# SaeedRahmani/MPC_for_AV_at_Intersection

Hardware: AMD Instinct MI355X
Metric: MPC timesteps/sec (whole node), N=20 horizon, 8-agent intersection, batch=4096 (higher is better)
Workload: dtype f64

## Files before the change

### mpc_for_av_at_intersection_amd/csrc/mpcx_prepare.hip

```cpp
#include "mpcx_common.h"
#include "mpcx_predict_core.h"
#include <cmath>

namespace mpcx {

struct RefArgs {
    mpcx_mpc_params p;
    int B;
    const double *state, *path, *path_v;
    const int32_t *path_off, *path_len;
    double dl;
    int32_t *target_ind;
    double *xref;
    uint8_t *re;
    const double *ov;
    long ov_stride;
    const int32_t *bin_cnt, *keyslot;
    int32_t *order;
    const int32_t *near, *near_tidx;
    const int32_t *stop_idx;
    double v_ref;
    int32_t *len_seen;
    const int32_t *done;
    int32_t *queue_len;
};

constexpr int PREP_WAVES = 4;
constexpr int WIN_AGENTS = 8;
static_assert(WIN_AGENTS <= WAVE, "one lane per agent in parts 1 and 2");
template <bool RETIRE>
__global__ __launch_bounds__(64 * PREP_WAVES) void ref_window_kernel(RefArgs a) {
    __shared__ int s_first[MPCX_ORDER_COPIES][MPCX_ORDER_BINS];
    const int lane = threadIdx.x & 63, wave = threadIdx.x >> 6;
    const int T = a.p.T, W = T + 1;
    const int b0 = ((int)blockIdx.x * PREP_WAVES + wave) * WIN_AGENTS;
    const int nag = a.B - b0 < WIN_AGENTS ? a.B - b0 : WIN_AGENTS;
    const bool own = lane < nag;
    const int b = own ? b0 + lane : 0;
    bool gone = !own;
    if constexpr (RETIRE) gone = gone || a.done[b] != 0;
    const int off = a.path_off[b], n = a.path_len[b];
    const double x = a.state[4 * b], y = a.state[4 * b + 1], v = a.state[4 * b + 2];
    const int start = a.target_ind[b];
    const int ks = a.order ? a.keyslot[b] : 0;
    const int hs = a.near ? a.near[3 * b] : -1, hm = a.near ? a.near[3 * b + 1] : -1, hl = a.near ? a.near[3 * b + 2] : -1;
    const int hint = a.near ? a.near_tidx[b] : -1;
    const int stop_at = a.stop_idx ? a.stop_idx[b] : MPCX_NO_STOP;
    if (a.order) {
        static_assert(MPCX_ORDER_BINS == 64, "one bin per lane");
        if (wave == 0) {
            int cnt[MPCX_ORDER_COPIES], c = 0;
#pragma unroll
            for (int q = 0; q < MPCX_ORDER_COPIES; q++) { cnt[q] = a.bin_cnt[q * MPCX_ORDER_BINS + lane]; c += cnt[q]; }
            int sfx = c;
#pragma unroll
            for (int d = 1; d < 64; d <<= 1) { const int o = __shfl_down(sfx, d); sfx += lane + d < 64 ? o : 0; }
            if constexpr (RETIRE) { if (blockIdx.x == 0 && lane == 0) *a.queue_len = sfx; }
            int first = sfx - c;
#pragma unroll
            for (int q = 0; q < MPCX_ORDER_COPIES; q++) { s_first[q][lane] = first; first += cnt[q]; }
        }
        __syncthreads();
        if (!gone)
            a.order[s_first[b % MPCX_ORDER_COPIES][(ks >> 24) & (MPCX_ORDER_BINS - 1)] + (ks & 0xFFFFFF)] = b;
    }
    int s = -1;
    bool scan = false;
    if (!gone) {
        if (hm >= 0 && start >= hs && hl >= start && hm < n) s = hint;
        else scan = !(start < 0 || n <= 0);
    }
    for (unsigned long long todo = __ballot(scan); todo; todo &= todo - 1) {
        const int i = __ffsll((long long)todo) - 1;
        const int r = nearest_index_in_direction(a.path + 3 * (size_t)__shfl(off, i), __shfl(n, i), __shfl(start, i), __shfl(x, i), __shfl(y, i), lane);
        s = lane == i ? r : s;
    }
    int stop = 0x7fffffff;
    if (!gone) {
        a.target_ind[b] = s;
        stop = stop_at == MPCX_NO_STOP ? stop : stop_at;
        if (a.stop_idx && a.len_seen) a.len_seen[b] = n;
    }
    const int G = 64 / W;
    const int g = lane / W, t = lane - g * W;
    for (int base = 0; base < nag; base += G) {
        const int i = base + g;
        const bool on = g < G && i < nag;
        const int from = on ? i : 0;
        const bool skip = __shfl((int)gone, from) != 0;
        const int si = __shfl(s, from), ni = __shfl(n, from), oi = __shfl(off, from), stopi = __shfl(stop, from);
        const double vi = __shfl(v, from);
        if (!on || skip) continue;
        const int bi = b0 + i;
        const double *path = a.path + 3 * (size_t)oi;
        const double *pv = a.path_v ? a.path_v + (size_t)oi : nullptr;
        double *xr = a.xref + (size_t)bi * 4 * W;
        uint8_t *re = a.re + (size_t)bi * W;
        if (si < 0) {
            xr[t] = 0; xr[W + t] = 0; xr[2 * W + t] = 0; xr[3 * W + t] = 0; re[t] = 0;
            continue;
        }
        const double ov = vi > 10.0 / 3.6 ? vi : 10.0 / 3.6;
        const double step = __dmul_rn(fabs(ov), a.p.dt);
        const double *ovp = a.ov ? a.ov + (size_t)bi * a.ov_stride : nullptr;
        double travel = ovp ? __dmul_rn(fabs(ovp[0]), a.p.dt) : step;
        for (int k = 1; k <= t; k++) travel = __dadd_rn(travel, ovp ? __dmul_rn(fabs(ovp[k]), a.p.dt) : step);
        long long idx = (long long)rint(__ddiv_rn(travel, a.dl)) + si;
        if (idx > ni - 1) idx = ni - 1;
        xr[0 * W + t] = path[3 * idx];
        xr[1 * W + t] = path[3 * idx + 1];
        xr[2 * W + t] = idx >= stopi ? 0.0 : (pv ? pv[idx] : a.v_ref);
        xr[3 * W + t] = path[3 * idx + 2];
        re[t] = (idx == ni - 1);
    }
}

__device__ __forceinline__ double plant_tan(const mpcx_mpc_params &p, double delta) {
    return tan(fmax(fmin(delta, p.max_steer), -p.max_steer));
}
__device__ __forceinline__ double plant_rate_xy(double v, double cs) {
#pragma clang fp contract(off)
    return v * cs;
}
__device__ __forceinline__ double plant_rate_th(const mpcx_mpc_params &p, double v, double tn) {
#pragma clang fp contract(off)
    return (v / p.L) * tn;
}
__device__ __forceinline__ double plant_euler(const mpcx_mpc_params &p, double acc, double rate) { return fma(rate, p.dt, acc); }
__device__ __forceinline__ double plant_speed(const mpcx_mpc_params &p, double v, double a) {
    return fmax(fmin(plant_euler(p, v, a), p.max_speed), p.min_speed);
}
__device__ __forceinline__ void plant_step(const mpcx_mpc_params &p, double &x, double &y, double &v, double &th,
                                           double a, double delta) {
    const double tn = plant_tan(p, delta);
    double s, c;
    sincos(th, &s, &c);
    x = plant_euler(p, x, plant_rate_xy(v, c));
    y = plant_euler(p, y, plant_rate_xy(v, s));
    th = plant_euler(p, th, plant_rate_th(p, v, tn));
    v = plant_speed(p, v, a);
}

struct RollArgs {
    mpcx_mpc_params p;
    int B;
    const double *state, *u_warm;
    double *xbar;
    const int32_t *done;
};

constexpr int ROLL_GROUP = 4, ROLL_BLOCK = 256, ROLL_AGENTS = ROLL_BLOCK / ROLL_GROUP;
static_assert(WAVE % ROLL_GROUP == 0 && ROLL_BLOCK % WAVE == 0, "whole groups per wavefront");
inline size_t rollout_lds(int T) { return ROLL_AGENTS * (4 * (size_t)(T + 1) + 1) * sizeof(double); }
__device__ __forceinline__ void rollout_group(const mpcx_mpc_params &p, double x, double y, double v, double th, const double *oa, int j, double *xb) {
    constexpr int G = ROLL_GROUP;
    const int T = p.T, W = T + 1;
    if (j == 0) { xb[0] = x; xb[W] = y; xb[2 * W] = v; xb[3 * W] = th; }
    const auto euler = [&](double acc, double rate) { return plant_euler(p, acc, rate); };
    const auto speed = [&](double vv, double acc) { return plant_speed(p, vv, acc); };
    for (int t0 = 0; t0 < T; t0 += G) {
        const int t = t0 + j;
        const bool in = t < T;
        const double ai = oa && in ? oa[t] : 0.0, di = oa && in ? oa[T + t] : 0.0;
        const double tn = plant_tan(p, di);
        const double v0 = v, th0 = th;
        const double vn = group_chain<G>(v, ai, j, speed);
        const double vt = group_prev<G>(vn, v0, j);
        const double thn = group_chain<G>(th, plant_rate_th(p, vt, tn), j, euler);
        const double tht = group_prev<G>(thn, th0, j);
        double s, c;
        sincos(tht, &s, &c);
        const double xn = group_chain<G>(x, plant_rate_xy(vt, c), j, euler);
        const double yn = group_chain<G>(y, plant_rate_xy(vt, s), j, euler);
        if (in) { xb[t + 1] = xn; xb[W + t + 1] = yn; xb[2 * W + t + 1] = vn; xb[3 * W + t + 1] = thn; }
    }
}
template <bool RETIRE>
__global__ __launch_bounds__(ROLL_BLOCK) void rollout_kernel(RollArgs a) {
    constexpr int G = ROLL_GROUP;
    extern __shared__ double s_roll[];
    const int T = a.p.T, W = T + 1;
    const int RS = 4 * W + 1;
    auto s_x = [&](int row) -> double * { return s_roll + (size_t)row * RS; };
    const int b0 = (int)blockIdx.x * ROLL_AGENTS;
    const int n = a.B - b0 < ROLL_AGENTS ? a.B - b0 : ROLL_AGENTS;
    const int r = (int)threadIdx.x / G, j = (int)threadIdx.x % G;
    bool gone = r >= n;
    if constexpr (RETIRE) gone = gone || a.done[b0 + r] != 0;
    if (j == 0) s_x(r)[4 * W] = gone ? 1.0 : 0.0;
    if (!gone) {
        const int b = b0 + r;
        double x = a.state[4 * b], y = a.state[4 * b + 1], v = a.state[4 * b + 2], th = a.state[4 * b + 3];
        rollout_group(a.p, x, y, v, th, a.u_warm ? a.u_warm + (size_t)b * 2 * T : nullptr, j, s_x(r));
    }
    __syncthreads();
    double *out = a.xbar + (size_t)b0 * 4 * W;
    for (int i = threadIdx.x; i < n * 4 * W; i += ROLL_BLOCK) {
        const int row = i / (4 * W);
        if (!RETIRE || s_x(row)[4 * W] == 0.0) out[i] = s_x(row)[i - row * 4 * W];
    }
}


struct PlantArgs {
    mpcx_mpc_params p;
    int B;
    double *state;
    double *u;
    const int32_t *status;
    double *applied;
    const mpcx_qp_tuning *tune;
    const int32_t *iters;
    unsigned long long *stats;
    int has_stats;
    int32_t *zero_bins, *zero_ticket;
    const int32_t *done;
};

__device__ __forceinline__ void plant_stats(unsigned long long *stats, int b, bool in, int it, bool bad) {
    int s_it = it, s_bad = bad ? 1 : 0, s_n = in ? 1 : 0, s_mx = it;
#pragma unroll
    for (int d = 32; d >= 1; d >>= 1) {
        s_it += __shfl_xor(s_it, d, WAVE); s_bad += __shfl_xor(s_bad, d, WAVE); s_n += __shfl_xor(s_n, d, WAVE);
        const int o = __shfl_xor(s_mx, d, WAVE); s_mx = o > s_mx ? o : s_mx;
    }
    if ((threadIdx.x & 63) == 0) {
        unsigned long long *w = stats + 4 * (size_t)(b >> 6);
        w[0] += (unsigned long long)s_n; w[1] += (unsigned long long)s_it; w[2] += (unsigned long long)s_bad;
        if ((unsigned long long)s_mx > w[3]) w[3] = (unsigned long long)s_mx;
    }
}

__global__ __launch_bounds__(256) void plant_kernel(PlantArgs a) {
    if (a.zero_bins && blockIdx.x == 0) {
        for (int i = threadIdx.x; i < MPCX_ORDER_COPIES * MPCX_ORDER_BINS; i += blockDim.x) a.zero_bins[i] = 0;
        if (threadIdx.x < MPCX_TICKET_WORDS) a.zero_ticket[threadIdx.x] = 0;
    }
    const int b = blockIdx.x * blockDim.x + threadIdx.x;
    const bool gone = a.done && b < a.B && a.done[b] != 0;
    if (a.has_stats) {
        const bool in = b < a.B && !gone;
        plant_stats(a.stats, b, in, in ? a.iters[b] : 0, in && a.status[b] != MPCX_QP_OPTIMAL);
    }
    if (b >= a.B || gone) return;
    const int T = a.p.T;
    double di = a.applied[2 * b], ai;
    const bool ok = !a.status || a.status[b] == MPCX_QP_OPTIMAL;
    if (ok) { di = a.u[(size_t)b * 2 * T + T]; ai = a.u[(size_t)b * 2 * T]; }
    else {
        ai = a.tune ? a.tune[b].max_decel : a.p.max_decel;
        for (int t = 0; t < 2 * T; t++) a.u[(size_t)b * 2 * T + t] = 0.0;
    }
    a.applied[2 * b] = di; a.applied[2 * b + 1] = ai;
    double x = a.state[4 * b], y = a.state[4 * b + 1], v = a.state[4 * b + 2], th = a.state[4 * b + 3];
    plant_step(a.p, x, y, v, th, ai, di);
    a.state[4 * b] = x; a.state[4 * b + 1] = y; a.state[4 * b + 2] = v; a.state[4 * b + 3] = th;
}

struct HeadArgs {
    mpcx_mpc_params p;
    mpcx_interaction_params ip;
    int B;
    double *state, *applied, *u;
    double *xbar, *obs6, *pred;
    const int32_t *status, *iters;
    const mpcx_qp_tuning *tune;
    unsigned long long *stats;
    int32_t *zero_bins, *zero_ticket;
};

constexpr int HEAD_BLOCK = ROLL_BLOCK + WAVE;
static_assert(ROLL_AGENTS == WAVE, "the prediction wavefront holds the workgroup's agents one per lane; its statistics slot is plant_kernel's");
template <bool PLANT>
__global__ __launch_bounds__(HEAD_BLOCK) void head_kernel(HeadArgs a) {
    constexpr int G = ROLL_GROUP;
    extern __shared__ double s_roll[];
    const int T = a.p.T, W = T + 1;
    const int RS = 4 * W + 1;
    const int tid = (int)threadIdx.x;
    const bool pred_wave = tid >= ROLL_BLOCK;
    const int b0 = (int)blockIdx.x * ROLL_AGENTS;
    const int n = a.B - b0 < ROLL_AGENTS ? a.B - b0 : ROLL_AGENTS;
    const int r = pred_wave ? tid - ROLL_BLOCK : tid / G, j = tid % G;
    const bool in = r < n;
    const int b = b0 + (in ? r : 0);
    double x = a.state[4 * b], y = a.state[4 * b + 1], v = a.state[4 * b + 2], th = a.state[4 * b + 3];
    double di = 0.0, ai = 0.0;
    bool failed = false;
    if constexpr (PLANT) {
        if (a.zero_bins && blockIdx.x == 0) {
            for (int i = tid; i < MPCX_ORDER_COPIES * MPCX_ORDER_BINS; i += HEAD_BLOCK) a.zero_bins[i] = 0;
            if (tid < MPCX_TICKET_WORDS) a.zero_ticket[tid] = 0;
        }
        failed = a.status[b] != MPCX_QP_OPTIMAL;
        const int it = pred_wave && in ? a.iters[b] : 0;
        di = a.applied[2 * b];
        if (!failed) { di = a.u[(size_t)b * 2 * T + T]; ai = a.u[(size_t)b * 2 * T]; }
        else { ai = a.p.max_decel; if (a.tune) ai = a.tune[b].max_decel; }
        plant_step(a.p, x, y, v, th, ai, di);
        __syncthreads();
        if (pred_wave) {
            plant_stats(a.stats, b0 + r, in, it, in && failed);
            if (in) {
                if (failed) for (int t = 0; t < 2 * T; t++) a.u[(size_t)b * 2 * T + t] = 0.0;
                a.applied[2 * b] = di; a.applied[2 * b + 1] = ai;
                a.state[4 * b] = x; a.state[4 * b + 1] = y; a.state[4 * b + 2] = v; a.state[4 * b + 3] = th;
            }
        }
    } else if (pred_wave) {
        di = a.applied[2 * b]; ai = a.applied[2 * b + 1];
    }
    if (pred_wave) {
        if (!in) return;
        double *row = a.obs6 + 6 * (size_t)b;
        row[0] = x; row[1] = y; row[2] = v; row[3] = th; row[4] = ai; row[5] = di;
        predict_row<false>(a.ip, x, y, v, th, ai, di, nullptr, a.pred + (size_t)b * a.ip.pred_steps * 4);
        return;
    }
    if (in) rollout_group(a.p, x, y, v, th, failed ? nullptr : a.u + (size_t)b * 2 * T, j, s_roll + (size_t)r * RS);
    __builtin_amdgcn_fence(__ATOMIC_RELEASE, "wavefront");
    __builtin_amdgcn_wave_barrier();
    __builtin_amdgcn_fence(__ATOMIC_ACQUIRE, "wavefront");
    constexpr int ROWS = WAVE / G;
    const int lane = tid & 63, r0 = (tid >> 6) * ROWS;
    const int nr = n - r0 < ROWS ? n - r0 : ROWS;
    double *out = a.xbar + (size_t)(b0 + r0) * 4 * W;
    for (int i = lane; i < nr * 4 * W; i += WAVE) {
        const int row = i / (4 * W);
        out[i] = s_roll[(size_t)(r0 + row) * RS + (i - row * 4 * W)];
    }
}

}

extern "C" int32_t mpcx_mpc_prepare_batch(mpcx_ctx *ctx, int32_t B, const double *state, const double *u_warm,
                                          const double *path_xyyaw, const double *path_v, const int32_t *path_off,
                                          const int32_t *path_len, double dl, int32_t *target_ind, double *xref, uint8_t *reaches_end, double *xbar) {
    return mpcx_mpc_prepare_batch_ov(ctx, B, state, u_warm, path_xyyaw, path_v, path_off, path_len, dl, target_ind, nullptr, 0, xref, reaches_end, xbar);
}

extern "C" int32_t mpcx_mpc_prepare_batch_ov(mpcx_ctx *ctx, int32_t B, const double *state, const double *u_warm,
                                             const double *path_xyyaw, const double *path_v, const int32_t *path_off,
                                             const int32_t *path_len, double dl, int32_t *target_ind, const double *ov, int64_t ov_stride,
                                             double *xref, uint8_t *reaches_end, double *xbar) {
    return mpcx_window_enqueue(ctx, B, state, u_warm, path_xyyaw, path_v, path_off, path_len, dl, target_ind, ov, ov_stride, xref, reaches_end, xbar, {});
}

extern "C" int32_t mpcx_mpc_prepare_batch_stop(mpcx_ctx *ctx, int32_t B, const double *state, const double *u_warm,
                                               const double *path_xyyaw, const double *path_v, const int32_t *path_off,
                                               const int32_t *path_len, double dl, int32_t *target_ind, const double *ov, int64_t ov_stride,
                                               const int32_t *stop_idx, double v_ref, int32_t *len_seen,
                                               double *xref, uint8_t *reaches_end, double *xbar) {
    mpcx_window_extras wx;
    wx.stop_idx = stop_idx; wx.v_ref = v_ref; wx.len_seen = len_seen;
    return mpcx_window_enqueue(ctx, B, state, u_warm, path_xyyaw, path_v, path_off, path_len, dl, target_ind, ov, ov_stride, xref, reaches_end, xbar, wx);
}

int32_t mpcx_window_enqueue(mpcx_ctx *ctx, int32_t B, const double *state, const double *u_warm, const double *path_xyyaw, const double *path_v,
                            const int32_t *path_off, const int32_t *path_len, double dl, int32_t *target_ind, const double *ov, int64_t ov_stride,
                            double *xref, uint8_t *reaches_end, double *xbar, const mpcx_window_extras &x) {
    if (!ctx) return MPCX_E_INVALID;
    if (!ctx->have_mpc) return mpcx_fail(ctx, MPCX_E_INVALID, "mpcx_set_mpc_params has not been called");
    if (B == 0) return MPCX_OK;
    if (B < 0 || !state || !path_xyyaw || !path_off || !path_len || !target_ind || !xref || !reaches_end || !xbar || !(dl > 0))
        return mpcx_fail(ctx, MPCX_E_INVALID, "mpc_prepare_batch: null pointer, negative batch or dl <= 0");
    if (ov && ov_stride < (int64_t)ctx->mpc.T + 1)
        return mpcx_fail(ctx, MPCX_E_INVALID, "mpc_prepare_batch_ov: ov_stride %lld is smaller than T + 1", (long long)ov_stride);
    if (x.stop_idx && !std::isfinite(x.v_ref))
        return mpcx_fail(ctx, MPCX_E_INVALID, "mpc_prepare_batch_stop: v_ref is not finite");
    mpcx::RefArgs ra{ctx->mpc, B, state, path_xyyaw, path_v, path_off, path_len, dl, target_ind, xref, reaches_end, ov, (long)ov_stride,
                     x.scatter ? ctx->bins : nullptr, x.scatter ? ctx->bins + MPCX_ORDER_COPIES * MPCX_ORDER_BINS : nullptr, x.scatter ? ctx->order : nullptr,
                     x.near, x.near ? x.tidx : nullptr, x.stop_idx, x.stop_idx ? x.v_ref : 0.0, x.stop_idx ? x.len_seen : nullptr,
                     x.done, x.queue_len};
    const bool retire = x.done != nullptr;
    if (retire && (!x.scatter || !x.queue_len))
        return mpcx_fail(ctx, MPCX_E_INVALID, "mpc_prepare_batch: retirement needs the queue order built beside the window selection");
    const bool forked = x.rollout_forked;
    if (x.rollout_done) {
        constexpr int per_block = mpcx::PREP_WAVES * mpcx::WIN_AGENTS;
        const dim3 wgrid((B + per_block - 1) / per_block), wblock(64 * mpcx::PREP_WAVES);
        if (retire) hipLaunchKernelGGL(mpcx::ref_window_kernel<true>, wgrid, wblock, 0, ctx->stream, ra);
        else hipLaunchKernelGGL(mpcx::ref_window_kernel<false>, wgrid, wblock, 0, ctx->stream, ra);
        return mpcx_check_launch(ctx, "prepare kernels");
    }
    if (!forked) {
        int32_t rc = mpcx_rollout_fork(ctx, B, state, u_warm, xbar, x.done);
        if (rc != MPCX_OK) return rc;
    }
    if (forked && hipStreamWaitEvent(ctx->stream, ctx->ev_join, 0) != hipSuccess)
        return mpcx_fail(ctx, MPCX_E_LAUNCH, "mpc_prepare_batch: cannot join the side stream");
    constexpr int per_block = mpcx::PREP_WAVES * mpcx::WIN_AGENTS;
    const dim3 wgrid((B + per_block - 1) / per_block), wblock(64 * mpcx::PREP_WAVES);
    if (retire) hipLaunchKernelGGL(mpcx::ref_window_kernel<true>, wgrid, wblock, 0, ctx->stream, ra);
    else hipLaunchKernelGGL(mpcx::ref_window_kernel<false>, wgrid, wblock, 0, ctx->stream, ra);
    if (!forked && hipStreamWaitEvent(ctx->stream, ctx->ev_join, 0) != hipSuccess)
        return mpcx_fail(ctx, MPCX_E_LAUNCH, "mpc_prepare_batch: cannot join the side stream");
    return mpcx_check_launch(ctx, "prepare kernels");
}

int32_t mpcx_rollout_fork(mpcx_ctx *ctx, int32_t B, const double *state, const double *u_warm, double *xbar, const int32_t *done) {
    mpcx::RollArgs ro{ctx->mpc, B, state, u_warm, xbar, done};
    if (hipEventRecord(ctx->ev_fork, ctx->stream) != hipSuccess || hipStreamWaitEvent(ctx->side, ctx->ev_fork, 0) != hipSuccess)
        return mpcx_fail(ctx, MPCX_E_LAUNCH, "mpc_prepare_batch: cannot fork the side stream");
    const size_t roll_lds = mpcx::rollout_lds(ctx->mpc.T);
    const dim3 rgrid((B + mpcx::ROLL_AGENTS - 1) / mpcx::ROLL_AGENTS), rblock(mpcx::ROLL_BLOCK);
    if (done) hipLaunchKernelGGL(mpcx::rollout_kernel<true>, rgrid, rblock, roll_lds, ctx->side, ro);
    else hipLaunchKernelGGL(mpcx::rollout_kernel<false>, rgrid, rblock, roll_lds, ctx->side, ro);
    const int32_t rc = mpcx_check_launch(ctx, "rollout_kernel");
    if (rc != MPCX_OK) return rc;
    if (hipEventRecord(ctx->ev_join, ctx->side) != hipSuccess)
        return mpcx_fail(ctx, MPCX_E_LAUNCH, "mpc_prepare_batch: cannot record the join event");
    return MPCX_OK;
}

int32_t mpcx_head_enqueue(mpcx_ctx *ctx, const mpcx_interaction_params *ip, int32_t P, double *state, double *applied, double *u,
                          const int32_t *status, const int32_t *iters, double *xbar, double *obs6, bool plant, bool reset_bins) {
    if (!ctx || !ip || P <= 0 || !state || !applied || !u || !status || !iters || !xbar || !obs6 || !ctx->pred || !ctx->stats)
        return mpcx_fail(ctx, MPCX_E_INVALID, "closed_loop_run: null pointer at the head of a step");
    if (ctx->pred_cap < (size_t)P * ip->pred_steps * 4 * sizeof(double) || ctx->stats_slots < ((size_t)P + 63) / 64)
        return mpcx_fail(ctx, MPCX_E_INVALID, "closed_loop_run: the prediction scratch or the statistics are too small for %d agents", P);
    if (ctx->tune && ctx->tune_rows != P)
        return mpcx_fail(ctx, MPCX_E_INVALID, "plant_step_batch: %d tuning rows are set but the batch has %d agents", ctx->tune_rows, P);
    const bool rz = plant && reset_bins && ctx->bins && ctx->ticket;
    mpcx::HeadArgs ha{ctx->mpc, *ip, P, state, applied, u, xbar, obs6, ctx->pred, status, iters, ctx->tune, ctx->stats,
                      rz ? ctx->bins : nullptr, rz ? ctx->ticket : nullptr};
    const size_t lds = mpcx::rollout_lds(ctx->mpc.T);
    const dim3 grid((P + mpcx::ROLL_AGENTS - 1) / mpcx::ROLL_AGENTS), block(mpcx::HEAD_BLOCK);
    if (plant) hipLaunchKernelGGL(mpcx::head_kernel<true>, grid, block, lds, ctx->stream, ha);
    else hipLaunchKernelGGL(mpcx::head_kernel<false>, grid, block, lds, ctx->stream, ha);
    return mpcx_check_launch(ctx, "head_kernel");
}

extern "C" int32_t mpcx_plant_step_batch(mpcx_ctx *ctx, int32_t B, double *state, double *u,
                                         const int32_t *status, double *applied) {
    return mpcx_plant_enqueue(ctx, B, state, u, status, applied, {});
}

int32_t mpcx_plant_enqueue(mpcx_ctx *ctx, int32_t B, double *state, double *u, const int32_t *status, double *applied, const mpcx_plant_extras &x) {
    if (!ctx) return MPCX_E_INVALID;
    if (!ctx->have_mpc) return mpcx_fail(ctx, MPCX_E_INVALID, "mpcx_set_mpc_params has not been called");
    if (B == 0) return MPCX_OK;
    if (B < 0 || !state || !u || !applied) return mpcx_fail(ctx, MPCX_E_INVALID, "plant_step_batch: null pointer");
    if (ctx->tune && ctx->tune_rows != B)
        return mpcx_fail(ctx, MPCX_E_INVALID, "plant_step_batch: %d tuning rows are set but the batch has %d agents", ctx->tune_rows, B);
    const bool st = ctx->stats && x.stats_iters && status;
    const bool rz = x.reset_bins && ctx->bins && ctx->ticket;
    mpcx::PlantArgs pa{ctx->mpc, B, state, u, status, applied, ctx->tune, x.stats_iters, ctx->stats, st ? 1 : 0,
                       rz ? ctx->bins : nullptr, rz ? ctx->ticket : nullptr, x.done};
    hipLaunchKernelGGL(mpcx::plant_kernel, dim3((B + 63) / 64), dim3(64), 0, ctx->stream, pa);
    return mpcx_check_launch(ctx, "plant_kernel");
}

extern "C" int32_t mpcx_closed_loop_stats(mpcx_ctx *ctx, int64_t *out4, int32_t reset) {
    if (!ctx || !out4) return MPCX_E_INVALID;
    out4[0] = out4[1] = out4[2] = out4[3] = 0;
    if (!ctx->stats || !ctx->stats_slots) return MPCX_OK;
    std::vector<unsigned long long> h(4 * ctx->stats_slots);
    if (hipMemcpyAsync(h.data(), ctx->stats, h.size() * sizeof(unsigned long long), hipMemcpyDeviceToHost, ctx->stream) != hipSuccess ||
        hipStreamSynchronize(ctx->stream) != hipSuccess)
        return mpcx_fail(ctx, MPCX_E_LAUNCH, "closed_loop_stats: copy failed");
    for (size_t w = 0; w < ctx->stats_slots; w++) {
        out4[0] += (int64_t)h[4 * w]; out4[1] += (int64_t)h[4 * w + 1]; out4[2] += (int64_t)h[4 * w + 2];
        if ((int64_t)h[4 * w + 3] > out4[3]) out4[3] = (int64_t)h[4 * w + 3];
    }
    if (reset && hipMemsetAsync(ctx->stats, 0, h.size() * sizeof(unsigned long long), ctx->stream) != hipSuccess)
        return mpcx_fail(ctx, MPCX_E_LAUNCH, "closed_loop_stats: reset failed");
    return MPCX_OK;
}

extern "C" int32_t mpcx_closed_loop_queue(mpcx_ctx *ctx, int32_t P, int32_t *order, int32_t *keyslot) {
    if (!ctx || !order || !keyslot || P < 0) return MPCX_E_INVALID;
    const size_t counters = (size_t)MPCX_ORDER_COPIES * MPCX_ORDER_BINS;
    if (!ctx->order || !ctx->bins || ctx->order_cap < (size_t)P * sizeof(int32_t) || ctx->bins_cap < (counters + (size_t)P) * sizeof(int32_t))
        return mpcx_fail(ctx, MPCX_E_INVALID, "closed_loop_queue: no closed loop has built a work queue for %d agents on this context", P);
    if (P == 0) return MPCX_OK;
    if (hipMemcpyAsync(order, ctx->order, (size_t)P * sizeof(int32_t), hipMemcpyDeviceToHost, ctx->stream) != hipSuccess ||
        hipMemcpyAsync(keyslot, ctx->bins + counters, (size_t)P * sizeof(int32_t), hipMemcpyDeviceToHost, ctx->stream) != hipSuccess ||
        hipStreamSynchronize(ctx->stream) != hipSuccess)
        return mpcx_fail(ctx, MPCX_E_LAUNCH, "closed_loop_queue: copy failed");
    return MPCX_OK;
}
```

Before: 9.283 million.

## Scan nearest path index for several agents concurrently in lane subgroups

Instead of having the whole wave scan each agent's path in turn, agents needing a nearest-index search are packed into lane groups of width 8 to 64 according to how many need it. Each group runs a prefetched top-3 search over the path with a DPP/shuffle argmin, and the result is redistributed to the owning lane. Trivially short ranges are resolved directly, and very long ranges still use the old whole-wave serial path. This cuts the serialized per-agent loop in the reference window kernel, at the cost of more register use and narrower parallelism per scan.

```diff
diff --git a/mpc_for_av_at_intersection_amd/csrc/mpcx_prepare.hip b/mpc_for_av_at_intersection_amd/csrc/mpcx_prepare.hip
--- a/mpc_for_av_at_intersection_amd/csrc/mpcx_prepare.hip
+++ b/mpc_for_av_at_intersection_amd/csrc/mpcx_prepare.hip
@@ -28,6 +28,70 @@
 constexpr int PREP_WAVES = 4;
 constexpr int WIN_AGENTS = 8;
 static_assert(WIN_AGENTS <= WAVE, "one lane per agent in parts 1 and 2");
+
+template <int CTRL>
+__device__ __forceinline__ void argmin_link_dpp(double &d, int &i) {
+    const double od = dpp_mov<CTRL>(d, d);
+    const int oi = __builtin_amdgcn_update_dpp(i, i, CTRL, 0xF, 0xF, false);
+    const bool take = (od < d) || (od == d && oi < i);
+    d = take ? od : d;
+    i = take ? oi : i;
+}
+__device__ __forceinline__ void group_argmin(double &d, int &i, int gw) {
+    argmin_link_dpp<0xB1>(d, i);
+    argmin_link_dpp<0x4E>(d, i);
+    argmin_link_dpp<0x141>(d, i);
+    if (gw > 8) argmin_link_dpp<0x140>(d, i);
+#pragma unroll
+    for (int s = 16; s <= 32; s <<= 1) {
+        if (gw > s) {
+            const double od = __shfl_xor(d, s, WAVE);
+            const int oi = __shfl_xor(i, s, WAVE);
+            const bool take = (od < d) || (od == d && oi < i);
+            d = take ? od : d;
+            i = take ? oi : i;
+        }
+    }
+}
+__device__ __forceinline__ int nearest_index_in_group(const double *path, int len, int start, double x, double y, int gl, int gw) {
+    const int L = len > 0 ? len : 0;
+    const double *p0 = path + 3 * (size_t)(L ? start : 0);
+    Top3 top;
+    constexpr int DEPTH = 4;
+    double bx[DEPTH], by[DEPTH];
+#pragma unroll
+    for (int k = 0; k < DEPTH; k++) {
+        const int i = k * gw + gl;
+        const double *q = p0 + 3 * (size_t)(i < L ? i : 0);
+        bx[k] = q[0]; by[k] = q[1];
+    }
+    for (int i0 = 0; i0 < L; i0 += DEPTH * gw) {
+        double nbx[DEPTH], nby[DEPTH];
+#pragma unroll
+        for (int k = 0; k < DEPTH; k++) {
+            const int i = i0 + (DEPTH + k) * gw + gl;
+            const double *q = p0 + 3 * (size_t)(i < L ? i : 0);
+            nbx[k] = q[0]; nby[k] = q[1];
+        }
+#pragma unroll
+        for (int k = 0; k < DEPTH; k++) {
+            const int i = i0 + k * gw + gl;
+            if (i < L) top.offer(bx[k], by[k], x, y, i);
+        }
+#pragma unroll
+        for (int k = 0; k < DEPTH; k++) { bx[k] = nbx[k]; by[k] = nby[k]; }
+    }
+    int bi[3];
+#pragma unroll
+    for (int r = 0; r < 3; r++) {
+        double d = top.d0; int ix = top.i0;
+        group_argmin(d, ix, gw);
+        bi[r] = ix;
+        if (top.i0 == ix) { top.d0 = top.d1; top.i0 = top.i1; top.d1 = top.d2; top.i1 = top.i2; top.d2 = INFINITY; top.i2 = 0x7fffffff; }
+    }
+    return three_nearest(bi, start);
+}
+constexpr int GROUP_SCAN_MAX = 512;
 template <bool RETIRE>
 __global__ __launch_bounds__(64 * PREP_WAVES) void ref_window_kernel(RefArgs a) {
     __shared__ int s_first[MPCX_ORDER_COPIES][MPCX_ORDER_BINS];
@@ -70,8 +134,25 @@
         if (hm >= 0 && start >= hs && hl >= start && hm < n) s = hint;
         else scan = !(start < 0 || n <= 0);
     }
-    for (unsigned long long todo = __ballot(scan); todo; todo &= todo - 1) {
-        const int i = __ffsll((long long)todo) - 1;
+    const int range = scan ? n - start : 0;
+    const bool tiny = scan && range <= 2, far = range > GROUP_SCAN_MAX;
+    if (tiny) s = range <= 1 ? start : start + 1;
+    const bool grouped = scan && !tiny && !far;
+    const unsigned todo = (unsigned)__ballot(grouped);
+    if (todo) {
+        const int k = __popc(todo);
+        const int sh = k > 4 ? 3 : k > 2 ? 4 : k > 1 ? 5 : 6, gw = 1 << sh;
+        unsigned m = todo;
+        for (int j = lane >> sh; j > 0; j--) m &= m - 1;
+        const int from = __ffs(m ? m : todo) - 1;
+        const int so = __shfl(off, from), sn = __shfl(n, from), ss = __shfl(start, from);
+        const double sx = __shfl(x, from), sy = __shfl(y, from);
+        const int r = nearest_index_in_group(a.path + 3 * (size_t)so, m ? sn - ss : 0, ss, sx, sy, lane & (gw - 1), gw);
+        const int got = __shfl(r, (__popc(todo & ((1u << (lane & 31)) - 1u)) << sh) & 63);
+        s = grouped ? got : s;
+    }
+    for (unsigned long long rest = __ballot(far); rest; rest &= rest - 1) {
+        const int i = __ffsll((long long)rest) - 1;
         const int r = nearest_index_in_direction(a.path + 3 * (size_t)__shfl(off, i), __shfl(n, i), __shfl(start, i), __shfl(x, i), __shfl(y, i), lane);
         s = lane == i ? r : s;
     }
```

Result: no change. 9.347 million (median of 6 runs) (+0.7%).
